# SamArgt/AudioSourceSep

Measured on NVIDIA B200. Metric: glow_log_prob_samples_per_s, higher is better.
Workload: dtype bf16

## Files before the change

audiosourcesep_b200/csrc/flow_kernels.cu:

```cuda
#include "kernels.h"

namespace asep {

namespace {

constexpr int kThreads = 128;

template <int C>
__device__ __forceinline__ void load_row(const float* __restrict__ p, float (&v)[C]) {
  if constexpr (C % 4 == 0) {
#pragma unroll
    for (int i = 0; i < C / 4; ++i) {
      float4 t = reinterpret_cast<const float4*>(p)[i];
      v[4 * i] = t.x; v[4 * i + 1] = t.y; v[4 * i + 2] = t.z; v[4 * i + 3] = t.w;
    }
  } else if constexpr (C % 2 == 0) {
#pragma unroll
    for (int i = 0; i < C / 2; ++i) {
      float2 t = reinterpret_cast<const float2*>(p)[i];
      v[2 * i] = t.x; v[2 * i + 1] = t.y;
    }
  } else {
#pragma unroll
    for (int i = 0; i < C; ++i) v[i] = p[i];
  }
}

template <int C>
__device__ __forceinline__ void store_row(float* __restrict__ p, const float (&v)[C]) {
  if constexpr (C % 4 == 0) {
#pragma unroll
    for (int i = 0; i < C / 4; ++i)
// ... 13 lines not shown
  for (int i = threadIdx.x; i < n; i += blockDim.x) smem[i] = sc[i];
  __syncthreads();
}

template <int C>
__device__ __forceinline__ void pre_apply(const float (&x)[C], float (&u)[C], const float* smem) {
  float a[C];
#pragma unroll
  for (int i = 0; i < C; ++i) a[i] = x[i] * smem[i] + smem[C + i];
  const float* Wm = smem + 2 * C;
#pragma unroll
  for (int o = 0; o < C; ++o) {
    float acc = 0.f;
#pragma unroll
    for (int i = 0; i < C; ++i) acc = fmaf(a[i], Wm[i * C + o], acc);
    u[o] = acc;
  }
}

__device__ __forceinline__ void accumulate_sample(double* acc, float v, long long pix, long long M, int HW) {
  const bool valid = pix < M;
  const int n = valid ? (int)(pix / HW) : -1;
  const int n0 = __shfl_sync(0xffffffffu, n, 0);
  const bool uniform = __all_sync(0xffffffffu, n == n0 || !valid);
  if (uniform) {
    float s = warp_sum(valid ? v : 0.f);
    if ((threadIdx.x & 31) == 0 && n0 >= 0) atomicAdd(acc + n0, (double)s);
  } else if (valid) {
    atomicAdd(acc + n, (double)v);
  }
}

struct GArg {
  const float* G; const float* const3; const float* c3;
  int n3p, nparts, H, W;
  long long part_stride;
};

template <int C>
__device__ __forceinline__ void gather_fwd_row(const GArg& g, long long p, float (&rv)[C]) {
  const int w = (int)(p % g.W), h = (int)((p / g.W) % g.H);
#pragma unroll
  for (int c = 0; c < C; ++c) rv[c] = __ldg(g.c3 + c);
#pragma unroll
  for (int tap = 0; tap < 9; ++tap) {
    const int dy = tap / 3 - 1, dx = tap % 3 - 1;
    const int hh = h + dy, ww = w + dx;
    if (hh < 0 || hh >= g.H || ww < 0 || ww >= g.W) continue;
    const long long pp = p + (long long)dy * g.W + dx;
    const float* base = g.G + (pp >> 7) * (128ll * g.n3p) + (pp & 127) * 4;
#pragma unroll
    for (int q = 0; q < C / 4; ++q) {
      const int col = tap * C + 4 * q;
      const float* src = base + (long long)(col >> 2) * 512;
      float4 t = __ldg(reinterpret_cast<const float4*>(src));
      for (int part = 1; part < g.nparts; ++part) {
        const float4 v = __ldg(reinterpret_cast<const float4*>(src + part * g.part_stride));
        t.x += v.x; t.y += v.y; t.z += v.z; t.w += v.w;
      }
      const float4 k = __ldg(reinterpret_cast<const float4*>(g.const3 + col));
      t.x += k.x; t.y += k.y; t.z += k.z; t.w += k.w;
      rv[4 * q] += t.x; rv[4 * q + 1] += t.y; rv[4 * q + 2] += t.z; rv[4 * q + 3] += t.w;
    }
  }
}

template <int Ch>
__device__ __forceinline__ void gather_bwd_row(const GArg& g, long long p, float (&gb)[Ch]) {
  const int w = (int)(p % g.W), h = (int)((p / g.W) % g.H);
#pragma unroll
  for (int c = 0; c < Ch; ++c) gb[c] = 0.f;
#pragma unroll
  for (int tap = 0; tap < 9; ++tap) {
// ... 300 lines not shown
    case 16: { constexpr int kC = 16; __VA_ARGS__; } break;                                  \
    case 32: { constexpr int kC = 32; __VA_ARGS__; } break;                                  \
    default: throw Error(ASEP_ERR_UNSUPPORTED, strfmt("channel count %d not built (2,4,8,16,32)", C)); \
  }

void launch_pre(const float* x, float* u, const float* sc, long long M, int C, cudaStream_t s) {
  if (M == 0) return;
  HbmScope prof(kHbmFlowStep, 8.0 * C * (double)M, s);
  DISPATCH_C(C, (k_pre<kC><<<cdiv(M, kThreads), kThreads, 0, s>>>(x, u, sc, M)));
  ASEP_LAUNCH_CHECK();
}

void launch_post_pre(const float* u, const float* r, float* out, const float* sc_next, double* acc, long long M,
                     int HW, int C, cudaStream_t s) {
  if (M == 0) return;
  HbmScope prof(kHbmFlowStep, 12.0 * C * (double)M, s);
  if (sc_next) {
    DISPATCH_C(C, (k_post_pre<kC, true><<<cdiv(M, kThreads), kThreads, 0, s>>>(u, r, out, sc_next, acc, M, HW)));
  } else {
    DISPATCH_C(C, (k_post_pre<kC, false><<<cdiv(M, kThreads), kThreads, 0, s>>>(u, r, out, nullptr, acc, M, HW)));
  }
  ASEP_LAUNCH_CHECK();
}

void launch_inv_step(const float* y, const float* r, float* x, const float* sc, double* acc, long long M, int HW,
                     int C, cudaStream_t s) {
  if (M == 0) return;
  HbmScope prof(kHbmFlowStep, 12.0 * C * (double)M, s);
  DISPATCH_C(C, (k_inv_step<kC><<<cdiv(M, kThreads), kThreads, 0, s>>>(y, r, x, sc, acc, M, HW)));
  ASEP_LAUNCH_CHECK();
}

namespace {
GArg to_arg(const GatherSrc& g) { return GArg{g.G, g.const3, g.c3, g.n3p, g.nparts, g.H, g.W, g.part_stride}; }
#define DISPATCH_CG(C, EXPR)                                                                           \
  do {                                                                                                 \
    switch (C) {                                                                                       \
      case 4: { constexpr int kC = 4; EXPR; } break;                                                   \
      case 8: { constexpr int kC = 8; EXPR; } break;                                                   \
      case 16: { constexpr int kC = 16; EXPR; } break;                                                 \
      default: ASEP_CHECK(false, ASEP_ERR_UNSUPPORTED, "fused gather: channel count %d", C);           \
    }                                                                                                  \
  } while (0)
}

bool fused_gather_supported(int C) { return C == 4 || C == 8 || C == 16; }

void launch_post_pre_g(const float* u, const GatherSrc& g, float* r_out, float* out, const float* sc_next, double* acc,
                       long long M, int HW, int C, cudaStream_t s) {
  if (M == 0) return;
  HbmScope prof(kHbmFlowStep, (r_out ? 16.0 : 12.0) * C * (double)M, s);
  const GArg a = to_arg(g);
  if (sc_next) {
    DISPATCH_CG(C, (k_post_pre<kC, true, true><<<cdiv(M, kThreads), kThreads, 0, s>>>(u, nullptr, out, sc_next, acc, M, HW, a, r_out)));
  } else {
    DISPATCH_CG(C, (k_post_pre<kC, false, true><<<cdiv(M, kThreads), kThreads, 0, s>>>(u, nullptr, out, nullptr, acc, M, HW, a, r_out)));
  }
  ASEP_LAUNCH_CHECK();
}

void launch_inv_step_g(const float* y, const GatherSrc& g, float* x, const float* sc, double* acc, long long M, int HW,
                       int C, cudaStream_t s) {
  if (M == 0) return;
  HbmScope prof(kHbmFlowStep, 12.0 * C * (double)M, s);
  const GArg a = to_arg(g);
  DISPATCH_CG(C, (k_inv_step<kC, true><<<cdiv(M, kThreads), kThreads, 0, s>>>(y, nullptr, x, sc, acc, M, HW, a)));
  ASEP_LAUNCH_CHECK();
// ... 89 lines not shown
```

audiosourcesep_b200/csrc/glow_model.cu:

```cuda
#include "glow_model.h"

#include <cmath>
#include <cstring>

namespace asep {

void DeviceArena::reserve(size_t bytes) {
  if (bytes <= cap_) { off_ = 0; return; }
  release();
  CUDA_CHECK(cudaMalloc(&base_, bytes));
  cap_ = bytes;
  off_ = 0;
}
void* DeviceArena::take(size_t bytes) {
  size_t al = (bytes + 255) & ~(size_t)255;
  ASEP_CHECK(off_ + al <= cap_, ASEP_ERR_STATE, "arena overflow (%zu + %zu > %zu)", off_, al, cap_);
  void* p = base_ + off_;
  off_ += al;
  return p;
}
void DeviceArena::release() {
  if (base_) cudaFree(base_);
  base_ = nullptr;
  cap_ = off_ = 0;
// ... 411 lines not shown
        const size_t mw = (size_t)N * levels_[b].H * levels_[b].W * (F / 32);
        for (int i = 0; i < K; ++i) {
          uint32_t* m1 = reinterpret_cast<uint32_t*>(get(mw));
          uint32_t* m2 = reinterpret_cast<uint32_t*>(get(mw));
          if (pass == 1) { work_.M1[b].push_back(m1); work_.M2[b].push_back(m2); }
        }
      }
      if (dumps) {
        const size_t dn = (size_t)N * levels_[b].H * levels_[b].W * F / 2;
        for (int i = 0; i < K; ++i) {
          __nv_bfloat16* d1 = reinterpret_cast<__nv_bfloat16*>(get(dn));
          __nv_bfloat16* d2 = reinterpret_cast<__nv_bfloat16*>(get(dn));
          if (pass == 1) { work_.D1[b].push_back(d1); work_.D2[b].push_back(d2); }
        }
      }
    }
    const size_t st0 = (size_t)M0 * levels_[0].C;
    float* z = get((size_t)N * Dl_);
    float* gz = get((size_t)N * Dl_);
    float *gA = get(st0), *gB = get(st0), *gr = get(st0), *gu = get(st0), *gxb = get(st0);
    double* acc = nullptr;
    if (pass == 0) need(2 * (size_t)N * sizeof(double)); else acc = arena_.take_n<double>(2 * (size_t)N);
    float *a1 = nullptr, *a2 = nullptr, *t1 = nullptr, *t2 = nullptr;
    NNScratchTC tc{};
    if (fp32) {
      a1 = get((size_t)M0 * F); a2 = get((size_t)M0 * F);
      if (save) { t1 = get((size_t)M0 * F); t2 = get((size_t)M0 * F); }
    } else {
      size_t gfl = 0;
      for (int b = 0; b < L; ++b)
        gfl = std::max(gfl, is_tcx() ? nn_tcx_g_floats((long long)N * levels_[b].H * levels_[b].W, levels_[b].C)
                                     : nn_tc_g_floats((long long)N * levels_[b].H * levels_[b].W, levels_[b].C));
      tc.G = get(gfl);
      if (save) {
        tc.mask1 = reinterpret_cast<uint32_t*>(get((size_t)M0 * (F / 32)));
        tc.mask2 = reinterpret_cast<uint32_t*>(get((size_t)M0 * (F / 32)));
      }
    }
    if (pass == 1) {
      work_.z = z; work_.gz = gz; work_.gA = gA; work_.gB = gB; work_.gr = gr; work_.gu = gu; work_.gxb = gxb;
      work_.acc_ld = acc; work_.acc_prior = acc + N;
      work_.a1 = a1; work_.a2 = a2; work_.t1 = t1; work_.t2 = t2; work_.tc = tc;
    }
  }
}

void GlowModel::nn_forward(int b, int k, const float* state, float* r, int N, bool save, cudaStream_t s) {
  const Level& lv = levels_[b];
  StepDerived& sd = step(b, k);
  if (precision_ == ASEP_PREC_FP32) {
    nn_fp32_forward(sd.w32, state, work_.a1, work_.a2, r, N, lv.H, lv.W, lv.C, cfg_.n_filters, s);
  } else {
    uint32_t *m1 = nullptr, *m2 = nullptr;
    if (save && !work_.M1.empty() && !work_.M1[b].empty()) { m1 = work_.M1[b][k]; m2 = work_.M2[b][k]; }
    if (is_tcx()) {
      nn_tcx_forward(sd.wtc, work_.tc, state, r, m1, m2, N, lv.H, lv.W, lv.C, s);
    } else {
      __nv_bfloat16 *d1 = nullptr, *d2 = nullptr;
      if (save && dumping_ && !work_.D1[b].empty()) { d1 = work_.D1[b][k]; d2 = work_.D2[b][k]; }
      nn_tc_forward(sd.wtc, work_.tc, state, r, m1, m2, N, lv.H, lv.W, lv.C, s, d1, d2);
    }
  }
}

bool GlowModel::fused_gather(int b) const { return is_tc() && fused_gather_supported(levels_[b].C); }

GatherSrc GlowModel::gather_src(int b, int k, int N, bool backward) {
  const Level& lv = levels_[b];
  return nn_tc_gather_src(step(b, k).wtc, work_.tc, backward, (long long)N * lv.H * lv.W, lv.H, lv.W, is_tcx());
}

void GlowModel::nn_backward(int b, int k, const float* state, const float* gr, float* gxb, int N, cudaStream_t s) {
  const Level& lv = levels_[b];
  StepDerived& sd = step(b, k);
  if (precision_ == ASEP_PREC_FP32) {
    nn_fp32_forward(sd.w32, state, work_.a1, work_.a2, work_.gxb , N, lv.H, lv.W, lv.C,
                    cfg_.n_filters, s);
    nn_fp32_backward(sd.w32, work_.a1, work_.a2, gr, work_.t1, work_.t2, gxb, N, lv.H, lv.W, lv.C, cfg_.n_filters, s);
  } else if (is_tcx()) {
    nn_tcx_forward(sd.wtc, work_.tc, state, work_.gxb , work_.tc.mask1, work_.tc.mask2, N, lv.H, lv.W,
                   lv.C, s);
    nn_tcx_backward(sd.wtc, work_.tc, gr, work_.tc.mask1, work_.tc.mask2, gxb, N, lv.H, lv.W, lv.C, s);
  } else {
    nn_tc_forward(sd.wtc, work_.tc, state, work_.gxb , work_.tc.mask1, work_.tc.mask2, N, lv.H, lv.W,
                  lv.C, s);
    nn_tc_backward(sd.wtc, work_.tc, gr, work_.tc.mask1, work_.tc.mask2, gxb, N, lv.H, lv.W, lv.C, s);
  }
}

void GlowModel::run_forward(const float* x, int N, bool save, cudaStream_t s, bool dumps) {
  require_prepared();
  ensure_work(N, save, dumps);
  dumping_ = dumps && work_.dumps;
  const int L = cfg_.L, K = cfg_.K;
  CUDA_CHECK(cudaMemsetAsync(work_.acc_ld, 0, 2 * (size_t)work_.N * sizeof(double), s));
  launch_squeeze(x, work_.X[0], N, cfg_.H, cfg_.W, cfg_.C, 1, cfg_.minval, cfg_.maxval, 0, s);
  for (int b = 0; b < L; ++b) {
    const Level& lv = levels_[b];
    const long long M = (long long)N * lv.H * lv.W;
    const int HW = lv.H * lv.W;
    auto ubuf = [&](int k) { return work_.save ? work_.U[b][k] : work_.U[b][k & 1]; };
    auto rbuf = [&](int k) { return work_.save ? work_.R[b][k] : work_.R[b][0]; };
// ... 236 lines not shown
```

audiosourcesep_b200/csrc/kernels.h:

```cpp
#pragma once
#include "common.cuh"

namespace asep {

inline int step_const_floats(int C) { return 2 * C + 2 * C * C; }

struct GatherSrc {
  const float* G = nullptr;
  const float* const3 = nullptr;
  const float* c3 = nullptr;
  int n3p = 0, nparts = 1, H = 0, W = 0;
  long long part_stride = 0;
};

void launch_pre(const float* x, float* u, const float* sc, long long M, int C, cudaStream_t s);
void launch_post_pre(const float* u, const float* r, float* out, const float* sc_next, double* acc, long long M,
                     int HW, int C, cudaStream_t s);
void launch_post_pre_g(const float* u, const GatherSrc& g, float* r_out, float* out, const float* sc_next, double* acc,
                       long long M, int HW, int C, cudaStream_t s);
void launch_inv_step_g(const float* y, const GatherSrc& g, float* x, const float* sc, double* acc, long long M, int HW,
                       int C, cudaStream_t s);
void launch_bwd_pre_g(const float* gu, const GatherSrc& g, float* gx, const float* sc, long long M, int C, cudaStream_t s);
bool fused_gather_supported(int C);
void launch_inv_step(const float* y, const float* r, float* x, const float* sc, double* acc, long long M, int HW,
                     int C, cudaStream_t s);
void launch_bwd_coupling(const float* gy, const float* u, const float* r, float* gr, float* gu, long long M, int C,
                         cudaStream_t s);
void launch_bwd_pre(const float* gu, const float* gxb, float* gx, const float* sc, long long M, int C, cudaStream_t s);
void launch_squeeze(const float* x, float* y, int N, int H, int W, int C, int mode, float p0, float p1, int inverse,
                    cudaStream_t s);
void launch_split_merge(float* o, float* z, float* next, int N, int H, int W, int C, int Cz, int nb, int CL,
                        int coff, long long Dl, int merge, cudaStream_t s);
void launch_prior(const float* z, const float* loc, const float* log_scale, double* acc, float* gz, int N, int D,
                  cudaStream_t s);
void launch_prior_sample(const float* eps, const float* loc, const float* log_scale, float* z, int N, int D,
                         cudaStream_t s);
void launch_finish(const double* acc, float* out, double add, double scale, int N, cudaStream_t s,
                   const double* dev_add = nullptr);
void launch_channel_stats(const float* x, double* mean_std, long long M, int C, cudaStream_t s);
void launch_scale(float* x, float a, long long n, cudaStream_t s);
void launch_actnorm(const float* x, const float* log_scale, const float* shift, float* y, long long M, int C,
// ... 30 lines not shown
```

audiosourcesep_b200/csrc/nn_tc.cu:

```cuda
#include "nn_tc_shared.cuh"

namespace asep {

namespace {

constexpr int kBarBytes4 = 256;
constexpr int kSmemBytes4 = kARegionBytes + kStages * kStageBytes + kBiasBytes + kBarBytes4;

template <bool kBwd, bool kSaveMask, bool kF16>
__global__ void __launch_bounds__(kThreadsTC2, 1) k_nn_tc4(const TCParams prm) {
  extern __shared__ __align__(1024) uint8_t smem[];
  if ((smem_u32(smem) & 1023u) != 0u) __trap();
  constexpr int S = kStages;
  uint8_t* sA = smem;
  uint8_t* sB = smem + kARegionBytes;
  float* sBias = reinterpret_cast<float*>(smem + kARegionBytes + S * kStageBytes);
  uint64_t* bars = reinterpret_cast<uint64_t*>(smem + kARegionBytes + S * kStageBytes + kBiasBytes);
  const uint32_t full0 = smem_u32(&bars[0]), empty0 = smem_u32(&bars[S]);
  const uint32_t a1_ready = smem_u32(&bars[2 * S]), accfull0 = smem_u32(&bars[2 * S + 1]);
  const uint32_t accfree_h0 = smem_u32(&bars[2 * S + 3]), panel0 = smem_u32(&bars[2 * S + 4]);
  const uint32_t cons0 = smem_u32(&bars[2 * S + 12]);
  uint32_t* tmem_slot = reinterpret_cast<uint32_t*>(&bars[2 * S + 16]);

  const int warp = threadIdx.x >> 5, lane = threadIdx.x & 31;
// ... 12 lines not shown
  }
  if (warp == 2) tmem_alloc(smem_u32(tmem_slot), kTmemCols);
  tc_fence_before();
  __syncthreads();
  tc_fence_after();
  const uint32_t tmem_base = *tmem_slot;
  const uint32_t img3_bytes = (uint32_t)prm.n3p * 128u;

  if (warp == 0) {
    if (lane == 0) {
      uint32_t stage = 0, phase = 0;
      const uint8_t* w1 = reinterpret_cast<const uint8_t*>(prm.wimg);
      const uint8_t* w2 = w1 + (size_t)2 * prm.k1_panels * kStageBytes;
      const uint8_t* w3 = w2 + (size_t)2 * kNumPanels * kStageBytes;
      auto push = [&](const uint8_t* src, uint32_t bytes) {
        mbar_wait(empty0 + 8 * stage, phase ^ 1);
        mbar_expect_tx(full0 + 8 * stage, bytes);
        bulk_g2s(smem_u32(sB + stage * kStageBytes), src, bytes, full0 + 8 * stage);
        if (++stage == (uint32_t)S) { stage = 0; phase ^= 1; }
      };
      for (int round = 0; round < prm.num_rounds; ++round) {
        for (int half = 1; half >= 0; --half)
          for (int kp = 0; kp < prm.k1_panels; ++kp) push(w1 + (size_t)(half * prm.k1_panels + kp) * kStageBytes, kStageBytes);
        for (int i = 0; i < 2 * kNumPanels; ++i) push(w2 + (size_t)i * kStageBytes, kStageBytes);
        for (int kp = 0; kp < kNumPanels; ++kp) push(w3 + (size_t)kp * img3_bytes, img3_bytes);
      }
    }
  } else if (warp == 1) {
    if (lane == 0) {
      uint32_t stage = 0, phase = 0;
      const uint32_t a_base = smem_u32(sA);
      constexpr uint32_t idesc256 = make_idesc(256);
      constexpr uint32_t idesc256h = kF16 ? make_idesc_f16(256) : make_idesc(256);
      const uint32_t idesc3 = kF16 ? make_idesc_f16(prm.n3p) : make_idesc(prm.n3p);
      auto kblock = [&](uint32_t d_tmem, int kp, int steps, uint32_t idesc, bool first) {
        mbar_wait(full0 + 8 * stage, phase);
        tc_fence_after();
        const uint64_t da = make_desc(a_base + kp * kPanelBytes);
        const uint64_t db = make_desc(smem_u32(sB + stage * kStageBytes));
        for (int k = 0; k < steps; ++k) umma_bf16(d_tmem, da + (uint64_t)(2 * k), db + (uint64_t)(2 * k), idesc, !(first && k == 0));
        umma_commit(empty0 + 8 * stage);
        if (++stage == (uint32_t)S) { stage = 0; phase ^= 1; }
      };
      const uint32_t h0 = tmem_base, h1 = tmem_base + 256u;
      for (int round = 0; round < prm.num_rounds; ++round) {
        mbar_wait(a1_ready, round & 1);
        tc_fence_after();
        for (int kp = 0; kp < prm.k1_panels; ++kp) kblock(h1, kp, min(4, prm.k1_steps - 4 * kp), idesc256, kp == 0);
        umma_commit(accfull0 + 8);
        if (round > 0) {
          mbar_wait(accfree_h0, (round - 1) & 1);
          tc_fence_after();
        }
        for (int kp = 0; kp < prm.k1_panels; ++kp) kblock(h0, kp, min(4, prm.k1_steps - 4 * kp), idesc256, kp == 0);
        umma_commit(accfull0);
        for (int p = 0; p < 4; ++p) mbar_wait(panel0 + 8 * p, 0);
        tc_fence_after();
        for (int kp = 0; kp < kNumPanels; ++kp) {
          if (kp >= 4) {
            mbar_wait(panel0 + 8 * kp, 0);
            tc_fence_after();
          }
          kblock(h0, kp, 4, idesc256h, kp == 0);
        }
        umma_commit(accfull0);
        for (int kp = 0; kp < kNumPanels; ++kp) {
          kblock(h1, kp, 4, idesc256h, kp == 0);
          if (kp < 4) umma_commit(cons0 + 8 * kp);
        }
        umma_commit(accfull0 + 8);
        for (int p = 0; p < 4; ++p) mbar_wait(panel0 + 8 * p, 1);
        tc_fence_after();
        for (int kp = 0; kp < kNumPanels; ++kp) {
          if (kp >= 4) {
            mbar_wait(panel0 + 8 * kp, 1);
            tc_fence_after();
          }
          kblock(h0, kp, 4, idesc3, kp == 0);
        }
        umma_commit(accfull0);
      }
    }
  } else {
    const int lq = warp & 3;
    const int ch = (warp - 2) >> 2;
    const int row = lq * 32 + lane;
    const int wtid = threadIdx.x - 64;
    const uint32_t t_lane = tmem_base + ((uint32_t)(lq * 32) << 16);
    uint8_t* stg = sA + kARegionBytes - ((kTileM * prm.n3p * 4 + 1023) & ~1023);
    const int k1_pad = prm.k1_steps * 16;
    float4 b1v = make_float4(0.f, 0.f, 0.f, 0.f), b2v = b1v;
    if constexpr (!kBwd) {
      if (wtid < kF / 4) {
        b1v = __ldg(reinterpret_cast<const float4*>(prm.bias1) + wtid);
        b2v = __ldg(reinterpret_cast<const float4*>(prm.bias2) + wtid);
        reinterpret_cast<float4*>(sBias)[wtid] = b1v;
// ... 109 lines not shown
              }
              if constexpr (kSaveMask) { if (hh) mkh[pp] = bits; else mkl[pp] = bits; }
            } else {
              const uint32_t bits = hh ? mkh[pp] : mkl[pp];
#pragma unroll
              for (int c2 = 0; c2 < 16; ++c2) {
                const float f0 = ((bits >> (2 * c2)) & 1u) ? __uint_as_float(v[pp & 1][2 * c2]) : 0.f;
                const float f1 = ((bits >> (2 * c2 + 1)) & 1u) ? __uint_as_float(v[pp & 1][2 * c2 + 1]) : 0.f;
                pk[c2] = pack_bf16(f0, f1);
              }
            }
            if (dump != nullptr && valid) {
#pragma unroll
              for (int c4 = 0; c4 < 4; ++c4) {
                uint32_t d[4];
#pragma unroll
                for (int q = 0; q < 4; ++q) {
                  if constexpr (!kF16) {
                    d[q] = pk[4 * c4 + q];
                  } else {
                    const float2 f = __half22float2(*reinterpret_cast<const __half2*>(&pk[4 * c4 + q]));
                    d[q] = pack_bf16(f.x, f.y);
                  }
                }
                *reinterpret_cast<uint4*>(dump + p * kF + j * 32 + c4 * 8) = make_uint4(d[0], d[1], d[2], d[3]);
              }
            }
            if (gemm == 1 && hh == 0) mbar_wait(cons0 + 8 * pn, round & 1);
            uint8_t* base = sA + pn * kPanelBytes + row * 128;
#pragma unroll
            for (int c4 = 0; c4 < 4; ++c4)
              *reinterpret_cast<uint4*>(base + (((ch * 4 + c4) ^ (row & 7)) << 4)) =
                  make_uint4(pk[4 * c4], pk[4 * c4 + 1], pk[4 * c4 + 2], pk[4 * c4 + 3]);
            if (hh == 0 ? pp == 3 : (pp & 1)) {
              fence_proxy_async();
              tc_fence_before();
              __syncwarp();
              if (lane == 0) {
                if (hh == 0) {
#pragma unroll
                  for (int q = 0; q < 4; ++q) mbar_arrive(panel0 + 8 * q);
                } else {
                  mbar_arrive(panel0 + 8 * (pn - 1));
                  mbar_arrive(panel0 + 8 * pn);
                }
              }
            }
          }
          if (gemm == 1 && hh == 0 && prefetch_regs && round + 1 < prm.num_rounds) prefetch_a1(round + 1);
        }
        if constexpr (kSaveMask) {
          if (valid) {
            uint4* mo = reinterpret_cast<uint4*>(mask + p * (kF / 32) + ch * 8);
            mo[0] = make_uint4(mkl[0], mkl[1], mkl[2], mkl[3]);
            mo[1] = make_uint4(mkh[0], mkh[1], mkh[2], mkh[3]);
          }
        }
        if constexpr (!kBwd) {
          named_bar_sync(1, kWorkers2);
          if (wtid < kF / 4) reinterpret_cast<float4*>(sBias)[wtid] = gemm == 0 ? b2v : b1v;
        }
        if (stamp) ts[1 + gemm] = clock64();
      }

      mbar_wait(accfull0, (uint32_t)(round + 2) & 1u);
      tc_fence_after();
      if (stamp) ts[3] = clock64();
      if (prefetch_regs && round + 1 < prm.num_rounds) store_a1();
      if (stamp) ts[4] = clock64();
      {
        uint8_t* stg_row = stg + (size_t)row * 16;
        for (int j = ch; j < prm.n3p / 16; j += 4) {
          uint32_t v[2][16];
          const bool two = j + 2 < prm.n3p / 16;
          tmem_ld16(t_lane + (uint32_t)(j * 16), v[0]);
          if (two) tmem_ld16(t_lane + (uint32_t)((j + 2) * 16), v[1]);
          tmem_ld_wait();
#pragma unroll
          for (int i = 0; i < 2; ++i) {
            if (i == 1 && !two) break;
#pragma unroll
            for (int c4 = 0; c4 < 4; ++c4)
              *reinterpret_cast<uint4*>(stg_row + (size_t)((j + 2 * i) * 4 + c4) * (kTileM * 16)) =
                  make_uint4(v[i][4 * c4], v[i][4 * c4 + 1], v[i][4 * c4 + 2], v[i][4 * c4 + 3]);
          }
        }
        tc_fence_before();
        arrive_warp(accfree_h0);
        fence_proxy_async();
        named_bar_sync(2, kWorkers2);
        if (wtid == 0) {
          if (tile * kTileM < prm.M)
            bulk_s2g(prm.out + tile * kTileM * prm.n3p, smem_u32(stg), (uint32_t)(kTileM * prm.n3p * 4));
        }
      }
      if (stamp) ts[5] = clock64();
    }
    if (wtid == 0) bulk_wait_all();
  }

  tc_fence_before();
  __syncthreads();
  if (warp == 2) tmem_dealloc(tmem_base, kTmemCols);
}

int g_num_sms = 0;

bool g_prof_on = false;
std::vector<TcProfToken> g_prof_recs, g_prof_pool;
double g_prof_flops = 0.0;
double g_next_flops = 0.0;


template <bool kBwd, bool kSaveMask, bool kF16>
void launch_tc4(const TCParams& prm, int grid, cudaStream_t s) {
  auto kern = k_nn_tc4<kBwd, kSaveMask, kF16>;
  static bool attr_set = false;
  if (!attr_set) {
    CUDA_CHECK(cudaFuncSetAttribute(kern, cudaFuncAttributeMaxDynamicSharedMemorySize, kSmemBytes4));
    attr_set = true;
  }
  const TcProfToken tok = nn_tc_prof_begin(s);
  kern<<<grid, kThreadsTC2, kSmemBytes4, s>>>(prm);
  ASEP_LAUNCH_CHECK();
  nn_tc_prof_end(tok, s, g_next_flops);
}
// ... 59 lines not shown
  rec.on = true;
  CUDA_CHECK(cudaEventRecord(rec.a, s));
  return rec;
}
void nn_tc_prof_end(const TcProfToken& rec, cudaStream_t s, double flops) {
  if (!rec.on) return;
  CUDA_CHECK(cudaEventRecord(rec.b, s));
  g_prof_recs.push_back(rec);
  g_prof_flops += flops;
}

void nn_tc_profile(int on) {
  g_prof_on = on != 0;
  if (g_prof_on) {
    for (auto& r : g_prof_recs) g_prof_pool.push_back(r);
    g_prof_recs.clear();
    g_prof_flops = 0.0;
  }
}
bool nn_tc_profile_enabled() { return g_prof_on; }
void nn_tc_profile_read(double* total_ms, long long* launches, double* flops) {
  double ms = 0.0;
  for (auto& r : g_prof_recs) {
    CUDA_CHECK(cudaEventSynchronize(r.b));
    float t = 0.f;
    CUDA_CHECK(cudaEventElapsedTime(&t, r.a, r.b));
    ms += t;
  }
  if (total_ms) *total_ms = ms;
  if (launches) *launches = (long long)g_prof_recs.size();
  if (flops) *flops = g_prof_flops;
}

GatherSrc nn_tc_gather_src(const NNWeightsTC& w, const NNScratchTC& sc, bool backward, long long M, int H, int W, bool split) {
  GatherSrc g;
  g.G = sc.G;
  g.const3 = backward ? nullptr : w.const3;
  g.c3 = backward ? nullptr : w.c3;
  g.n3p = backward ? w.bwd.n3p : w.fwd.n3p;
  g.H = H; g.W = W;
  g.nparts = split ? 2 : 1;
  g.part_stride = split ? (M + kTileM - 1) / kTileM * kTileM * (long long)g.n3p : 0;
  return g;
}

size_t nn_tc_g_floats(long long M, int C) { return (size_t)((M + kTileM - 1) / kTileM * kTileM) * (size_t)pad16(9 * C); }

void nn_tc_prepare(NNWeightsTC& w, const float* k1, const float* c1, const float* g1, const float* b1,
                   const float* k2, const float* c2, const float* g2, const float* b2, const float* k3,
                   const float* c3, int C, int F, bool f16, bool x3) {
  ASEP_CHECK(F == kF, ASEP_ERR_UNSUPPORTED, "the tcgen05 coupling kernel is built for n_filters = %d (got %d)", kF, F);
  nn_tc_release(w);
  const int Ch = C / 2;
  {
    const int K1h = 9 * Ch;
    auto f1 = [&](int n, int k) { return k1[(size_t)(k % K1h) * F + n]; };
    auto f2 = [&](int n, int k) { return g1[k] * k2[(size_t)k * F + n]; };
    auto f3 = [&](int n, int k) {
      const int tap = n / C, c = n % C;
      return g2[k] * k3[((size_t)tap * F + k) * C + c];
    };
    const float ws = (f16 && x3) ? 256.f : 1.f;
    build_stage_set(w.fwd, 2 * K1h, 9 * C, f1, f2, f3,  f16,  f16 && x3, false, ws);
    if (x3) build_stage_set(w.fwd_lo, 2 * K1h, 9 * C, f1, f2, f3, f16, f16,  true, ws);
    w.wscale_fwd = ws;
  }
  {
    const int K1h = 9 * C;
    auto f1 = [&](int n, int k) {
      const int kk = k % K1h, tap = kk / C, c = kk % C;
      return g2[n] * k3[((size_t)tap * F + n) * C + c];
    };
    auto f2 = [&](int n, int k) { return g1[n] * k2[(size_t)n * F + k]; };
    auto f3 = [&](int n, int k) { return k1[(size_t)n * F + k]; };
    build_stage_set(w.bwd, 2 * K1h, 9 * Ch, f1, f2, f3, false);
    if (x3) build_stage_set(w.bwd_lo, 2 * K1h, 9 * Ch, f1, f2, f3, false, false,  true);
  }
// ... 10 lines not shown
      const3[(size_t)tap * C + c] = (float)a;
    }
  w.bias1 = upload(bias1);
  w.bias2 = upload(bias2);
  w.const3 = upload(const3);
  w.c3 = upload(vc3);
  w.f16 = f16;
  w.x3 = x3;
}

void nn_tc_release(NNWeightsTC& w) {
  if (w.fwd.img) cudaFree(w.fwd.img);
  if (w.bwd.img) cudaFree(w.bwd.img);
  if (w.fwd_lo.img) cudaFree(w.fwd_lo.img);
  if (w.bwd_lo.img) cudaFree(w.bwd_lo.img);
  if (w.bias1) cudaFree(w.bias1);
  if (w.bias2) cudaFree(w.bias2);
  if (w.const3) cudaFree(w.const3);
  if (w.c3) cudaFree(w.c3);
  w = NNWeightsTC{};
}

void nn_tc_forward(const NNWeightsTC& w, const NNScratchTC& sc, const float* state, float* r, uint32_t* mask1,
                   uint32_t* mask2, int N, int H, int W, int C, cudaStream_t s, __nv_bfloat16* dump1,
                   __nv_bfloat16* dump2) {
  const long long M = (long long)N * H * W;
  if (M == 0) return;
  TCParams prm{};
  prm.src = state; prm.src_stride = C; prm.src_off = C / 2; prm.src_ch = C / 2; prm.tap_sign = 1;
  prm.wimg = w.fwd.img; prm.k1_steps = w.fwd.k1_steps; prm.k1_panels = w.fwd.k1_panels; prm.n3p = w.fwd.n3p;
  prm.bias1 = w.bias1; prm.bias2 = w.bias2; prm.mask1 = mask1; prm.mask2 = mask2;
  prm.dump1 = dump1; prm.dump2 = dump2; prm.f16 = w.f16 ? 1 : 0;
  prm.out = sc.G; prm.H = H; prm.W = W; prm.M = M;
  g_next_flops = 2.0 * (double)M * (9.0 * (C / 2) * kF + (double)kF * kF + 9.0 * kF * C);
  run_tc<false>(prm, s);
  if (r != nullptr) launch_gather_fwd(sc.G, w.const3, w.c3, r, M, H, W, C, w.fwd.n3p, 1, 0, s);
}

void nn_tc_backward(const NNWeightsTC& w, const NNScratchTC& sc, const float* gr, const uint32_t* mask1,
                    const uint32_t* mask2, float* gxb, int N, int H, int W, int C, cudaStream_t s,
                    __nv_bfloat16* dump_gp2, __nv_bfloat16* dump_gp1) {
  const long long M = (long long)N * H * W;
  if (M == 0) return;
  TCParams prm{};
  prm.src = gr; prm.src_stride = C; prm.src_off = 0; prm.src_ch = C; prm.tap_sign = -1;
  prm.wimg = w.bwd.img; prm.k1_steps = w.bwd.k1_steps; prm.k1_panels = w.bwd.k1_panels; prm.n3p = w.bwd.n3p;
  prm.bias1 = nullptr; prm.bias2 = nullptr;
  prm.mask1 = const_cast<uint32_t*>(mask1); prm.mask2 = const_cast<uint32_t*>(mask2);
  prm.dump1 = dump_gp2; prm.dump2 = dump_gp1;
  prm.out = sc.G; prm.H = H; prm.W = W; prm.M = M;
  g_next_flops = 2.0 * (double)M * (9.0 * (C / 2) * kF + (double)kF * kF + 9.0 * kF * C);
  run_tc<true>(prm, s);
  if (gxb != nullptr) launch_gather_bwd(sc.G, gxb, M, H, W, C / 2, w.bwd.n3p, 1, 0, s);
}

}
```

audiosourcesep_b200/csrc/nn_tc.h:

```cpp
#pragma once
#include <vector>
#include "common.cuh"
#include "kernels.h"

namespace asep {

constexpr int kTcF = 512;

struct TCStageSet {
  __nv_bfloat16* img = nullptr;
  int k1_steps = 0;
  int k1_panels = 0;
  int n3p = 0;
  size_t bytes = 0;
};

struct NNWeightsTC {
  TCStageSet fwd, bwd;
  TCStageSet fwd_lo, bwd_lo;
  bool x3 = false;
  float wscale_fwd = 1.f;
  float* bias1 = nullptr;
  float* bias2 = nullptr;
  float* const3 = nullptr;
  float* c3 = nullptr;
  bool f16 = false;
};

struct NNScratchTC {
  float* G = nullptr;
  uint32_t* mask1 = nullptr;
  uint32_t* mask2 = nullptr;
};

void nn_tc_prepare(NNWeightsTC& w, const float* k1, const float* c1, const float* g1, const float* b1,
                   const float* k2, const float* c2, const float* g2, const float* b2, const float* k3,
                   const float* c3, int C, int F, bool f16 = false, bool x3 = false);
void nn_tc_release(NNWeightsTC& w);

void nn_tc_forward(const NNWeightsTC& w, const NNScratchTC& sc, const float* state, float* r, uint32_t* mask1,
                   uint32_t* mask2, int N, int H, int W, int C, cudaStream_t s, __nv_bfloat16* dump1 = nullptr,
                   __nv_bfloat16* dump2 = nullptr);
void nn_tc_backward(const NNWeightsTC& w, const NNScratchTC& sc, const float* gr, const uint32_t* mask1,
                    const uint32_t* mask2, float* gxb, int N, int H, int W, int C, cudaStream_t s,
                    __nv_bfloat16* dump_gp2 = nullptr, __nv_bfloat16* dump_gp1 = nullptr);

size_t nn_tc_g_floats(long long M, int C);
GatherSrc nn_tc_gather_src(const NNWeightsTC& w, const NNScratchTC& sc, bool backward, long long M, int H, int W, bool split);

void nn_tcx_forward(const NNWeightsTC& w, const NNScratchTC& sc, const float* state, float* r, uint32_t* mask1,
                    uint32_t* mask2, int N, int H, int W, int C, cudaStream_t s);
void nn_tcx_backward(const NNWeightsTC& w, const NNScratchTC& sc, const float* gr, const uint32_t* mask1,
                     const uint32_t* mask2, float* gxb, int N, int H, int W, int C, cudaStream_t s);
size_t nn_tcx_g_floats(long long M, int C);
void nn_tc_profile(int on);
struct TcProfToken { cudaEvent_t a = nullptr, b = nullptr; bool on = false; };
TcProfToken nn_tc_prof_begin(cudaStream_t s);
void nn_tc_prof_end(const TcProfToken& tok, cudaStream_t s, double flops);
bool nn_tc_profile_enabled();
void nn_tc_profile_read(double* total_ms, long long* launches, double* flops);

}
```

audiosourcesep_b200/csrc/nn_tc_shared.cuh:

```cuda
#pragma once
#include "nn_tc.h"
#include "tc_ptx.cuh"

#include <cmath>
#include <cstring>

namespace asep {
namespace {

constexpr int kF = kTcF;
constexpr int kTileM = 128;
constexpr int kPanelBytes = kTileM * 128;
constexpr int kNumPanels = kF / 64;
constexpr int kARegionBytes = kNumPanels * kPanelBytes;
constexpr int kStageRows = 256;
constexpr int kStageBytes = kStageRows * 128;
constexpr int kStages = 3;
constexpr int kBiasBytes = kF * 4;
constexpr int kTmemCols = 512;

struct TCParams {
  const float* src;
  int src_stride;
  int src_off;
  int src_ch;
  int tap_sign;
  const __nv_bfloat16* wimg;
  const __nv_bfloat16* wimg_lo;
  int f16_s1;
  float acc_scale;
  int k1_steps, k1_panels, n3p;
  const float* bias1;
  const float* bias2;
  uint32_t* mask1;
  uint32_t* mask2;
  float* out;
  int H, W;
  long long M;
  __nv_bfloat16* dump1;
  __nv_bfloat16* dump2;
  long long* dbg_out;
  int f16;
  long long part_stride;
  int tiles_per_cta_round;
  int num_rounds;
};

__device__ __forceinline__ uint32_t a_offset(int row, int k) {
  return (uint32_t)((k >> 6) * kPanelBytes + row * 128 + ((((k & 63) >> 3) ^ (row & 7)) << 4) + ((k & 7) << 1));
}


constexpr int kThreadsTC2 = 64 + 256;
constexpr int kWorkers2 = 256;

template <bool kHalf>
__device__ __forceinline__ void split_pair(float a, float b, uint32_t& hi, uint32_t& lo) {
  if constexpr (kHalf) {
    __half2 h = __floats2half2_rn(a, b);
    const float2 hf = __half22float2(h);
    __half2 l = __floats2half2_rn(a - hf.x, b - hf.y);
    hi = *reinterpret_cast<uint32_t*>(&h);
    lo = *reinterpret_cast<uint32_t*>(&l);
  } else {
    __nv_bfloat162 h = __floats2bfloat162_rn(a, b);
    hi = *reinterpret_cast<uint32_t*>(&h);
    __nv_bfloat162 l = __floats2bfloat162_rn(a - __uint_as_float(hi << 16), b - __uint_as_float(hi & 0xffff0000u));
    lo = *reinterpret_cast<uint32_t*>(&l);
  }
// ... 203 lines not shown
      }
      if constexpr (kFwd) {
        const float4 k = __ldg(reinterpret_cast<const float4*>(const3 + col));
        t.x += k.x; t.y += k.y; t.z += k.z; t.w += k.w;
      }
      acc[0] += t.x; acc[1] += t.y; acc[2] += t.z; acc[3] += t.w;
    } else {
      float2 t = __ldg(reinterpret_cast<const float2*>(g));
      for (int q = 1; q < nparts; ++q) {
        const float2 u = __ldg(reinterpret_cast<const float2*>(g + q * part_stride));
        t.x += u.x; t.y += u.y;
      }
      if constexpr (kFwd) {
        const float2 k = __ldg(reinterpret_cast<const float2*>(const3 + col));
        t.x += k.x; t.y += k.y;
      }
      acc[0] += t.x; acc[1] += t.y;
    }
  }
  if constexpr (V == 4) reinterpret_cast<float4*>(out)[idx] = make_float4(acc[0], acc[1], acc[2], acc[3]);
  else reinterpret_cast<float2*>(out)[idx] = make_float2(acc[0], acc[1]);
}

inline int pad16(int n) { return (n + 15) / 16 * 16; }

inline void launch_gather_fwd(const float* G, const float* const3, const float* c3, float* r, long long M, int H, int W, int C,
                              int n3p, int nparts, long long part_stride, cudaStream_t s) {
  const long long total = M * C;
  HbmScope prof(kHbmGather, 4.0 * (9.0 * C * nparts + C) * (double)M, s);
  if (C % 4 == 0) k_gather_vec<4, true><<<cdiv(total / 4, 256), 256, 0, s>>>(G, const3, c3, r, H, W, C, n3p, total / 4, nparts, part_stride);
  else k_gather_fwd<true><<<cdiv(total, 256), 256, 0, s>>>(G, const3, c3, r, H, W, C, n3p, total, nparts, part_stride);
  ASEP_LAUNCH_CHECK();
}
inline void launch_gather_bwd(const float* G, float* gxb, long long M, int H, int W, int Ch, int n3p, int nparts,
                              long long part_stride, cudaStream_t s) {
  const long long total = M * Ch;
  HbmScope prof(kHbmGather, 4.0 * (9.0 * Ch * nparts + Ch) * (double)M, s);
  if (Ch % 4 == 0) k_gather_vec<4, false><<<cdiv(total / 4, 256), 256, 0, s>>>(G, nullptr, nullptr, gxb, H, W, Ch, n3p, total / 4, nparts, part_stride);
  else if (Ch % 2 == 0) k_gather_vec<2, false><<<cdiv(total / 2, 256), 256, 0, s>>>(G, nullptr, nullptr, gxb, H, W, Ch, n3p, total / 2, nparts, part_stride);
  else k_gather_bwd<true><<<cdiv(total, 256), 256, 0, s>>>(G, gxb, H, W, Ch, n3p, total, nparts, part_stride);
  ASEP_LAUNCH_CHECK();
}

template <typename Fn>
void write_image(std::vector<__nv_bfloat16>& dst, int rows, int n0, int n_valid, int k0, int k_valid, Fn&& get, bool f16 = false,
                 bool lo_part = false, float wscale = 1.f) {
  const size_t base = dst.size();
  dst.resize(base + (size_t)rows * 64, __float2bfloat16(0.f));
  for (int r = 0; r < rows; ++r) {
    for (int k = 0; k < 64; ++k) {
      float v = 0.f;
      if (r < n_valid && k < k_valid) v = get(n0 + r, k0 + k) * wscale;
      const size_t off = (size_t)r * 64 + (size_t)((((k >> 3) ^ (r & 7)) << 3) + (k & 7));
      uint16_t bits;
      if (f16) {
        ASEP_CHECK(std::fabs(v) < 60000.f, ASEP_ERR_UNSUPPORTED, "coupling-network weight %g outside the fp16 range of this precision mode", v);
        __half hv = __float2half(v);
        if (lo_part) hv = __float2half(v - __half2float(hv));
        std::memcpy(&bits, &hv, sizeof(bits));
      } else {
        __nv_bfloat16 bv = __float2bfloat16(v);
        if (lo_part) bv = __float2bfloat16(v - __bfloat162float(bv));
        std::memcpy(&bits, &bv, sizeof(bits));
      }
      std::memcpy(reinterpret_cast<uint16_t*>(dst.data()) + base + off, &bits, sizeof(bits));
    }
// ... 35 lines not shown
```

Measured before the change: 19040.

## Fold 3x3 conv tap reduction into tensor-core kernel epilogue via compact records

In the forward tensor-core NN kernel, instead of bulk-storing the full per-tap partial matrix G (9*C columns per pixel) to global memory, worker threads reduce the taps within each 128-pixel tile in shared memory. They write a compact record holding the per-pixel partial sums plus three halo rows per tile. The downstream gather (standalone or fused into the flow-step kernels) then reads one float4 per channel group plus at most two halo terms, rather than nine taps. This cuts global traffic for the conv3 output. The cost is extra ALU work and a loop of non-bulk stores in the epilogue, which may lengthen the tensor-core pipeline, and it only applies when W divides 128 and C is 4, 8 or 16.

```diff
diff --git a/audiosourcesep_b200/csrc/conv3_rec.cuh b/audiosourcesep_b200/csrc/conv3_rec.cuh
--- /dev/null
+++ b/audiosourcesep_b200/csrc/conv3_rec.cuh
@@ -0,0 +1,75 @@
+#pragma once
+#include "common.cuh"
+
+namespace asep {
+namespace {
+
+constexpr int kRecTile = 128;
+
+inline bool conv3_rec_ok(int W, int C) { return W > 0 && W <= kRecTile && kRecTile % W == 0 && (C == 4 || C == 8 || C == 16); }
+inline size_t conv3_rec_floats(long long M, int W, int C) {
+  return (size_t)((M + kRecTile - 1) / kRecTile) * (size_t)(kRecTile + 3 * W) * (size_t)C;
+}
+
+__device__ __forceinline__ float4 add4(float4 a, float4 b) { return make_float4(a.x + b.x, a.y + b.y, a.z + b.z, a.w + b.w); }
+
+__device__ __forceinline__ float4 conv3_rec_unit(const uint8_t* stg, const float* __restrict__ const3, const float* __restrict__ c3,
+                                                 uint32_t p0, int slot, int cb, int C, int H, int W) {
+  const int C4 = C >> 2, R = kRecTile / W;
+  auto term = [&](int i, int tap) {
+    const float4 g = *reinterpret_cast<const float4*>(stg + ((tap * C4 + cb) * kRecTile + i) * 16);
+    return add4(g, __ldg(reinterpret_cast<const float4*>(const3 + tap * C) + cb));
+  };
+  auto row_sum = [&](int src_row, int dy, int w) {
+    const int t0 = (dy + 1) * 3, i = src_row * W + w;
+    float4 s = term(i, t0 + 1);
+    if (w > 0) s = add4(term(i - 1, t0), s);
+    if (w < W - 1) s = add4(s, term(i + 1, t0 + 2));
+    return s;
+  };
+  if (slot >= kRecTile) {
+    const int k = (slot - kRecTile) / W, w = slot - kRecTile - k * W;
+    if (k == 0) return R > 1 ? row_sum(1, 1, w) : make_float4(0.f, 0.f, 0.f, 0.f);
+    if (k == 1) return row_sum(0, 1, w);
+    return row_sum(R - 1, -1, w);
+  }
+  const int rr = slot / W, w = slot - rr * W;
+  const int h = (int)(((p0 + (uint32_t)slot) / (uint32_t)W) % (uint32_t)H);
+  const bool top = h > 0, bot = h < H - 1;
+  if (rr == 0 && top) return row_sum(0, 0, w);
+  float4 a = __ldg(reinterpret_cast<const float4*>(c3) + cb);
+  if (top) a = add4(a, row_sum(rr - 1, -1, w));
+  a = add4(a, row_sum(rr, 0, w));
+  if (bot && rr < R - 1) a = add4(a, row_sum(rr + 1, 1, w));
+  return a;
+}
+
+template <int C>
+__device__ __forceinline__ void conv3_rec_row(const float* __restrict__ rec, const float* __restrict__ c3, long long p, int H, int W,
+                                              float (&rv)[C]) {
+  const uint32_t pu = (uint32_t)p, i = pu & (kRecTile - 1);
+  const int S = kRecTile + 3 * W, R = kRecTile / W;
+  const int rr = (int)i / W, w = (int)i - rr * W;
+  const int h = (int)((pu / (uint32_t)W) % (uint32_t)H);
+  const bool up = rr == 0 && h > 0, down = rr == R - 1 && h < H - 1;
+  const float* t = rec + (long long)(pu / kRecTile) * S * C;
+  const long long tile = (long long)S * C;
+#pragma unroll
+  for (int q = 0; q < C / 4; ++q) {
+    const float* col = t + (long long)q * S * 4;
+    const float4 m = __ldg(reinterpret_cast<const float4*>(col) + i);
+    float4 a;
+    if (!up) {
+      a = m;
+    } else {
+      a = add4(__ldg(reinterpret_cast<const float4*>(c3) + q), __ldg(reinterpret_cast<const float4*>(col - tile) + kRecTile + 2 * W + w));
+      a = add4(a, m);
+    }
+    if (down) a = add4(a, __ldg(reinterpret_cast<const float4*>(col + tile) + kRecTile + W + w));
+    else if (up && h < H - 1) a = add4(a, __ldg(reinterpret_cast<const float4*>(col) + kRecTile + w));
+    rv[4 * q] = a.x; rv[4 * q + 1] = a.y; rv[4 * q + 2] = a.z; rv[4 * q + 3] = a.w;
+  }
+}
+
+}
+}
diff --git a/audiosourcesep_b200/csrc/flow_kernels.cu b/audiosourcesep_b200/csrc/flow_kernels.cu
--- a/audiosourcesep_b200/csrc/flow_kernels.cu
+++ b/audiosourcesep_b200/csrc/flow_kernels.cu
@@ -1,3 +1,4 @@
+#include "conv3_rec.cuh"
 #include "kernels.h"
 
 namespace asep {
@@ -77,13 +78,17 @@
 }
 
 struct GArg {
-  const float* G; const float* const3; const float* c3;
+  const float* G; const float* rec; const float* const3; const float* c3;
   int n3p, nparts, H, W;
   long long part_stride;
 };
 
 template <int C>
 __device__ __forceinline__ void gather_fwd_row(const GArg& g, long long p, float (&rv)[C]) {
+  if (g.rec != nullptr) {
+    conv3_rec_row<C>(g.rec, g.c3, p, g.H, g.W, rv);
+    return;
+  }
   const int w = (int)(p % g.W), h = (int)((p / g.W) % g.H);
 #pragma unroll
   for (int c = 0; c < C; ++c) rv[c] = __ldg(g.c3 + c);
@@ -450,7 +455,7 @@
 }
 
 namespace {
-GArg to_arg(const GatherSrc& g) { return GArg{g.G, g.const3, g.c3, g.n3p, g.nparts, g.H, g.W, g.part_stride}; }
+GArg to_arg(const GatherSrc& g) { return GArg{g.G, g.rec, g.const3, g.c3, g.n3p, g.nparts, g.H, g.W, g.part_stride}; }
 #define DISPATCH_CG(C, EXPR)                                                                           \
   do {                                                                                                 \
     switch (C) {                                                                                       \
diff --git a/audiosourcesep_b200/csrc/glow_model.cu b/audiosourcesep_b200/csrc/glow_model.cu
--- a/audiosourcesep_b200/csrc/glow_model.cu
+++ b/audiosourcesep_b200/csrc/glow_model.cu
@@ -467,6 +467,12 @@
         gfl = std::max(gfl, is_tcx() ? nn_tcx_g_floats((long long)N * levels_[b].H * levels_[b].W, levels_[b].C)
                                      : nn_tc_g_floats((long long)N * levels_[b].H * levels_[b].W, levels_[b].C));
       tc.G = get(gfl);
+      if (!is_tcx()) {
+        size_t rfl = 0;
+        for (int b = 0; b < L; ++b)
+          rfl = std::max(rfl, nn_tc_rec_floats((long long)N * levels_[b].H * levels_[b].W, levels_[b].W, levels_[b].C));
+        if (rfl > 0) tc.rec = get(rfl);
+      }
       if (save) {
         tc.mask1 = reinterpret_cast<uint32_t*>(get((size_t)M0 * (F / 32)));
         tc.mask2 = reinterpret_cast<uint32_t*>(get((size_t)M0 * (F / 32)));
@@ -502,7 +508,7 @@
 
 GatherSrc GlowModel::gather_src(int b, int k, int N, bool backward) {
   const Level& lv = levels_[b];
-  return nn_tc_gather_src(step(b, k).wtc, work_.tc, backward, (long long)N * lv.H * lv.W, lv.H, lv.W, is_tcx());
+  return nn_tc_gather_src(step(b, k).wtc, work_.tc, backward, (long long)N * lv.H * lv.W, lv.H, lv.W, lv.C, is_tcx());
 }
 
 void GlowModel::nn_backward(int b, int k, const float* state, const float* gr, float* gxb, int N, cudaStream_t s) {
diff --git a/audiosourcesep_b200/csrc/kernels.h b/audiosourcesep_b200/csrc/kernels.h
--- a/audiosourcesep_b200/csrc/kernels.h
+++ b/audiosourcesep_b200/csrc/kernels.h
@@ -7,6 +7,7 @@
 
 struct GatherSrc {
   const float* G = nullptr;
+  const float* rec = nullptr;
   const float* const3 = nullptr;
   const float* c3 = nullptr;
   int n3p = 0, nparts = 1, H = 0, W = 0;
diff --git a/audiosourcesep_b200/csrc/nn_tc.cu b/audiosourcesep_b200/csrc/nn_tc.cu
--- a/audiosourcesep_b200/csrc/nn_tc.cu
+++ b/audiosourcesep_b200/csrc/nn_tc.cu
@@ -328,11 +328,22 @@
         }
         tc_fence_before();
         arrive_warp(accfree_h0);
-        fence_proxy_async();
-        named_bar_sync(2, kWorkers2);
-        if (wtid == 0) {
-          if (tile * kTileM < prm.M)
-            bulk_s2g(prm.out + tile * kTileM * prm.n3p, smem_u32(stg), (uint32_t)(kTileM * prm.n3p * 4));
+        if (kBwd || prm.rec == nullptr) {
+          fence_proxy_async();
+          named_bar_sync(2, kWorkers2);
+          if (wtid == 0) {
+            if (tile * kTileM < prm.M)
+              bulk_s2g(prm.out + tile * kTileM * prm.n3p, smem_u32(stg), (uint32_t)(kTileM * prm.n3p * 4));
+          }
+        } else {
+          named_bar_sync(2, kWorkers2);
+          if (tile * kTileM < prm.M) {
+            const int C = 2 * prm.src_ch, S = kTileM + 3 * prm.W, units = S * (C >> 2);
+            float4* dst = reinterpret_cast<float4*>(prm.rec + tile * (long long)units * 4);
+#pragma unroll 1
+            for (int u = wtid; u < units; u += kWorkers2)
+              dst[u] = conv3_rec_unit(stg, prm.const3, prm.c3, (uint32_t)(tile * kTileM), u % S, u / S, C, prm.H, prm.W);
+          }
         }
       }
       if (stamp) ts[5] = clock64();
@@ -458,9 +469,10 @@
   if (flops) *flops = g_prof_flops;
 }
 
-GatherSrc nn_tc_gather_src(const NNWeightsTC& w, const NNScratchTC& sc, bool backward, long long M, int H, int W, bool split) {
+GatherSrc nn_tc_gather_src(const NNWeightsTC& w, const NNScratchTC& sc, bool backward, long long M, int H, int W, int C, bool split) {
   GatherSrc g;
   g.G = sc.G;
+  g.rec = !backward && !split && nn_tc_uses_rec(sc, W, C) ? sc.rec : nullptr;
   g.const3 = backward ? nullptr : w.const3;
   g.c3 = backward ? nullptr : w.c3;
   g.n3p = backward ? w.bwd.n3p : w.fwd.n3p;
@@ -469,6 +481,9 @@
   g.part_stride = split ? (M + kTileM - 1) / kTileM * kTileM * (long long)g.n3p : 0;
   return g;
 }
+
+bool nn_tc_uses_rec(const NNScratchTC& sc, int W, int C) { return sc.rec != nullptr && conv3_rec_ok(W, C); }
+size_t nn_tc_rec_floats(long long M, int W, int C) { return conv3_rec_ok(W, C) ? conv3_rec_floats(M, W, C) : 0; }
 
 size_t nn_tc_g_floats(long long M, int C) { return (size_t)((M + kTileM - 1) / kTileM * kTileM) * (size_t)pad16(9 * C); }
 
@@ -545,9 +560,14 @@
   prm.bias1 = w.bias1; prm.bias2 = w.bias2; prm.mask1 = mask1; prm.mask2 = mask2;
   prm.dump1 = dump1; prm.dump2 = dump2; prm.f16 = w.f16 ? 1 : 0;
   prm.out = sc.G; prm.H = H; prm.W = W; prm.M = M;
+  const bool rec = nn_tc_uses_rec(sc, W, C);
+  if (rec) { prm.rec = sc.rec; prm.const3 = w.const3; prm.c3 = w.c3; }
   g_next_flops = 2.0 * (double)M * (9.0 * (C / 2) * kF + (double)kF * kF + 9.0 * kF * C);
   run_tc<false>(prm, s);
-  if (r != nullptr) launch_gather_fwd(sc.G, w.const3, w.c3, r, M, H, W, C, w.fwd.n3p, 1, 0, s);
+  if (r != nullptr) {
+    if (rec) launch_rec_fwd(sc.rec, w.c3, r, M, H, W, C, s);
+    else launch_gather_fwd(sc.G, w.const3, w.c3, r, M, H, W, C, w.fwd.n3p, 1, 0, s);
+  }
 }
 
 void nn_tc_backward(const NNWeightsTC& w, const NNScratchTC& sc, const float* gr, const uint32_t* mask1,
diff --git a/audiosourcesep_b200/csrc/nn_tc.h b/audiosourcesep_b200/csrc/nn_tc.h
--- a/audiosourcesep_b200/csrc/nn_tc.h
+++ b/audiosourcesep_b200/csrc/nn_tc.h
@@ -29,6 +29,7 @@
 
 struct NNScratchTC {
   float* G = nullptr;
+  float* rec = nullptr;
   uint32_t* mask1 = nullptr;
   uint32_t* mask2 = nullptr;
 };
@@ -46,7 +47,10 @@
                     __nv_bfloat16* dump_gp2 = nullptr, __nv_bfloat16* dump_gp1 = nullptr);
 
 size_t nn_tc_g_floats(long long M, int C);
-GatherSrc nn_tc_gather_src(const NNWeightsTC& w, const NNScratchTC& sc, bool backward, long long M, int H, int W, bool split);
+size_t nn_tc_rec_floats(long long M, int W, int C);
+bool nn_tc_uses_rec(const NNScratchTC& sc, int W, int C);
+GatherSrc nn_tc_gather_src(const NNWeightsTC& w, const NNScratchTC& sc, bool backward, long long M, int H, int W, int C,
+                           bool split);
 
 void nn_tcx_forward(const NNWeightsTC& w, const NNScratchTC& sc, const float* state, float* r, uint32_t* mask1,
                     uint32_t* mask2, int N, int H, int W, int C, cudaStream_t s);
diff --git a/audiosourcesep_b200/csrc/nn_tc_shared.cuh b/audiosourcesep_b200/csrc/nn_tc_shared.cuh
--- a/audiosourcesep_b200/csrc/nn_tc_shared.cuh
+++ b/audiosourcesep_b200/csrc/nn_tc_shared.cuh
@@ -1,4 +1,5 @@
 #pragma once
+#include "conv3_rec.cuh"
 #include "nn_tc.h"
 #include "tc_ptx.cuh"
 
@@ -35,6 +36,9 @@
   uint32_t* mask1;
   uint32_t* mask2;
   float* out;
+  float* rec;
+  const float* const3;
+  const float* c3;
   int H, W;
   long long M;
   __nv_bfloat16* dump1;
@@ -304,6 +308,28 @@
   else k_gather_fwd<true><<<cdiv(total, 256), 256, 0, s>>>(G, const3, c3, r, H, W, C, n3p, total, nparts, part_stride);
   ASEP_LAUNCH_CHECK();
 }
+template <int C>
+__global__ void __launch_bounds__(256) k_rec_to_r(const float* __restrict__ rec, const float* __restrict__ c3, float* __restrict__ r,
+                                                  int H, int W, long long M) {
+  const long long p = (long long)blockIdx.x * blockDim.x + threadIdx.x;
+  if (p >= M) return;
+  float rv[C];
+  conv3_rec_row<C>(rec, c3, p, H, W, rv);
+#pragma unroll
+  for (int q = 0; q < C / 4; ++q) reinterpret_cast<float4*>(r + p * C)[q] = make_float4(rv[4 * q], rv[4 * q + 1], rv[4 * q + 2], rv[4 * q + 3]);
+}
+
+inline void launch_rec_fwd(const float* rec, const float* c3, float* r, long long M, int H, int W, int C, cudaStream_t s) {
+  HbmScope prof(kHbmGather, 8.0 * C * (double)M, s);
+  switch (C) {
+    case 4: k_rec_to_r<4><<<cdiv(M, 256), 256, 0, s>>>(rec, c3, r, H, W, M); break;
+    case 8: k_rec_to_r<8><<<cdiv(M, 256), 256, 0, s>>>(rec, c3, r, H, W, M); break;
+    case 16: k_rec_to_r<16><<<cdiv(M, 256), 256, 0, s>>>(rec, c3, r, H, W, M); break;
+    default: ASEP_CHECK(false, ASEP_ERR_UNSUPPORTED, "conv3 record: channel count %d", C);
+  }
+  ASEP_LAUNCH_CHECK();
+}
+
 inline void launch_gather_bwd(const float* G, float* gxb, long long M, int H, int W, int Ch, int n3p, int nparts,
                               long long part_stride, cudaStream_t s) {
   const long long total = M * Ch;
```

New measurement: 19780, median of 6. 3.9% higher.

## Start second GEMM on first A panels before all four panels ready

Applied to the files above, without the earlier changes.

The MMA warp now waits only for panels 0 and 1 before issuing the first two K-blocks of the second GEMM as N=128 half-width MMAs into the low accumulator half. It keeps those weight stages held, then waits for panels 2 and 3 and issues the matching upper-half N=128 MMAs before releasing the stages. On the producer side, the four-panel batch signal is limited to gemm 1, so later epilogues signal panels in pairs. The aim is to overlap the epilogue that writes the A panels with the tensor-core work, at the cost of more MMA instructions and more complex stage and barrier handling.

```diff
diff --git a/audiosourcesep_b200/csrc/nn_tc.cu b/audiosourcesep_b200/csrc/nn_tc.cu
--- a/audiosourcesep_b200/csrc/nn_tc.cu
+++ b/audiosourcesep_b200/csrc/nn_tc.cu
@@ -68,15 +68,21 @@
       const uint32_t a_base = smem_u32(sA);
       constexpr uint32_t idesc256 = make_idesc(256);
       constexpr uint32_t idesc256h = kF16 ? make_idesc_f16(256) : make_idesc(256);
+      constexpr uint32_t idesc128h = kF16 ? make_idesc_f16(128) : make_idesc(128);
       const uint32_t idesc3 = kF16 ? make_idesc_f16(prm.n3p) : make_idesc(prm.n3p);
-      auto kblock = [&](uint32_t d_tmem, int kp, int steps, uint32_t idesc, bool first) {
+      auto next_slot = [&]() {
         mbar_wait(full0 + 8 * stage, phase);
         tc_fence_after();
-        const uint64_t da = make_desc(a_base + kp * kPanelBytes);
-        const uint64_t db = make_desc(smem_u32(sB + stage * kStageBytes));
+        const uint32_t s = stage;
+        if (++stage == (uint32_t)S) { stage = 0; phase ^= 1; }
+        return s;
+      };
+      auto slot_desc = [&](uint32_t s) { return make_desc(smem_u32(sB + s * kStageBytes)); };
+      auto kblock = [&](uint32_t d_tmem, int kp, int steps, uint32_t idesc, bool first) {
+        const uint32_t s = next_slot();
+        const uint64_t da = make_desc(a_base + kp * kPanelBytes), db = slot_desc(s);
         for (int k = 0; k < steps; ++k) umma_bf16(d_tmem, da + (uint64_t)(2 * k), db + (uint64_t)(2 * k), idesc, !(first && k == 0));
-        umma_commit(empty0 + 8 * stage);
-        if (++stage == (uint32_t)S) { stage = 0; phase ^= 1; }
+        umma_commit(empty0 + 8 * s);
       };
       const uint32_t h0 = tmem_base, h1 = tmem_base + 256u;
       for (int round = 0; round < prm.num_rounds; ++round) {
@@ -90,14 +96,32 @@
         }
         for (int kp = 0; kp < prm.k1_panels; ++kp) kblock(h0, kp, min(4, prm.k1_steps - 4 * kp), idesc256, kp == 0);
         umma_commit(accfull0);
-        for (int p = 0; p < 4; ++p) mbar_wait(panel0 + 8 * p, 0);
+        mbar_wait(panel0, 0);
+        mbar_wait(panel0 + 8, 0);
         tc_fence_after();
-        for (int kp = 0; kp < kNumPanels; ++kp) {
+        uint32_t held[2];
+#pragma unroll
+        for (int kp = 0; kp < 2; ++kp) {
+          held[kp] = next_slot();
+          const uint64_t da = make_desc(a_base + kp * kPanelBytes), db = slot_desc(held[kp]);
+          for (int k = 0; k < 4; ++k) umma_bf16(h0, da + (uint64_t)(2 * k), db + (uint64_t)(2 * k), idesc128h, kp + k > 0);
+        }
+        mbar_wait(panel0 + 16, 0);
+        mbar_wait(panel0 + 24, 0);
+        tc_fence_after();
+#pragma unroll
+        for (int kp = 0; kp < 2; ++kp) {
+          const uint64_t da = make_desc(a_base + kp * kPanelBytes);
+          const uint64_t db = slot_desc(held[kp]) + (uint64_t)((128 * 128) >> 4);
+          for (int k = 0; k < 4; ++k) umma_bf16(h0 + 128u, da + (uint64_t)(2 * k), db + (uint64_t)(2 * k), idesc128h, kp + k > 0);
+          umma_commit(empty0 + 8 * held[kp]);
+        }
+        for (int kp = 2; kp < kNumPanels; ++kp) {
           if (kp >= 4) {
             mbar_wait(panel0 + 8 * kp, 0);
             tc_fence_after();
           }
-          kblock(h0, kp, 4, idesc256h, kp == 0);
+          kblock(h0, kp, 4, idesc256h, false);
         }
         umma_commit(accfull0);
         for (int kp = 0; kp < kNumPanels; ++kp) {
@@ -273,12 +297,13 @@
             for (int c4 = 0; c4 < 4; ++c4)
               *reinterpret_cast<uint4*>(base + (((ch * 4 + c4) ^ (row & 7)) << 4)) =
                   make_uint4(pk[4 * c4], pk[4 * c4 + 1], pk[4 * c4 + 2], pk[4 * c4 + 3]);
-            if (hh == 0 ? pp == 3 : (pp & 1)) {
+            const bool all4 = gemm == 1 && hh == 0;
+            if (all4 ? pp == 3 : (pp & 1)) {
               fence_proxy_async();
               tc_fence_before();
               __syncwarp();
               if (lane == 0) {
-                if (hh == 0) {
+                if (all4) {
 #pragma unroll
                   for (int q = 0; q < 4; ++q) mbar_arrive(panel0 + 8 * q);
                 } else {
```

After: 19120 before, 19180 after, median of 6. No clear change (+0.3%).
